# auduno/headtrackr

Hardware: AMD Instinct MI355X
Metric: frames/sec full-cascade detect at 320x240 (higher is better)
Workload: dtype u8; 1 GPU; C2: 256 x 320x240 RGBA frames per GPU, full BBF cascade detect (interval 5) incl. grouping + best face per frame on the host; frames_per_gpu=256, frames_total=256, width=320, height=240, batches_in_flight=3, parallelism=1 GPU

## Files before the change

headtrackr_amd/csrc/ht_context.hip:

```cpp
#include <sched.h>
#include <algorithm>
#include <cmath>
#include <cstddef>
#include <cstdlib>
#include <cstring>
#include <new>

#include "ht_internal.h"
#include "ht_hostpost.h"
#include "ht_geometry_plan.h"
#include "ht_cascade_plan.h"

static thread_local std::string g_create_err;

#include <dlfcn.h>
namespace {
struct Roctx {
    int (*push)(const char *) = nullptr;
    int (*pop)() = nullptr;
    Roctx() {
        void *h = dlopen("libroctx64.so", RTLD_NOW | RTLD_GLOBAL);
        if (!h) h = dlopen("libroctx64.so.4", RTLD_NOW | RTLD_GLOBAL);
        if (h) {
            push = reinterpret_cast<int (*)(const char *)>(dlsym(h, "roctxRangePushA"));
// ... 69 lines not shown
        int cpus = sched_getaffinity(0, sizeof(set), &set) == 0 ? CPU_COUNT(&set) : (int)std::thread::hardware_concurrency();
        int ngpu = 1;
        if (hipGetDeviceCount(&ngpu) != hipSuccess || ngpu < 1) ngpu = 1;
        return std::max(0, std::min(7, cpus / (2 * ngpu) - 1));
    }();
    return share;
}


ht_status ht_fail(ht_ctx *ctx, ht_status st, const std::string &msg) {
    if (ctx)
        ctx->err = msg;
    else
        g_create_err = msg;
    return st;
}

HtProfScope::HtProfScope(ht_ctx *c, const char *name, hipStream_t on) : ctx(c), stream(on ? on : c->stream) {
    if (!ctx->profiling) return;
    for (size_t i = 0; i < ctx->timers.size(); i++)
        if (ctx->timers[i].name == name) idx = (int)i;
    if (idx < 0) {
        ctx->timers.emplace_back();
        ctx->timers.back().name = name;
        idx = (int)ctx->timers.size() - 1;
    }
    if (hipEventCreate(&a) != hipSuccess || hipEventCreate(&b) != hipSuccess) {
        idx = -1;
        return;
    }
    (void)hipEventRecord(a, stream);
}
HtProfScope::~HtProfScope() {
    if (idx < 0) return;
    (void)hipEventRecord(b, stream);
    ctx->timers[idx].pending.emplace_back(a, b);
    ctx->timers[idx].launches++;
}

extern "C" int32_t ht_abi_version(void) { return HT_ABI_VERSION; }

extern "C" const char *ht_last_error(const ht_ctx *ctx) { return ctx ? ctx->err.c_str() : g_create_err.c_str(); }

static bool apply_options(ht_ctx *c, const std::string &opts, std::string &why) {
    size_t pos = 0;
    while (pos < opts.size()) {
        size_t end = opts.find(',', pos);
        if (end == std::string::npos) end = opts.size();
        std::string kv = opts.substr(pos, end - pos);
        pos = end + 1;
        while (!kv.empty() && (kv.front() == ' ')) kv.erase(kv.begin());
        while (!kv.empty() && (kv.back() == ' ')) kv.pop_back();
        if (kv.empty()) continue;
        const size_t eq = kv.find('=');
        const std::string key = kv.substr(0, eq), val = eq == std::string::npos ? "1" : kv.substr(eq + 1);
        char *endp = nullptr;
        const long long v = std::strtoll(val.c_str(), &endp, 10);
        if (val.empty() || (endp && *endp)) {
            why = "option '" + key + "': value is not an integer";
            return false;
        }
        const int iv = (int)std::max<long long>(std::min<long long>(v, 1ll << 30), -(1ll << 30));
        if (key == "rs_rpt") { if (iv >= 1 && iv <= HT_RS_MAX_PASSES) c->rs_rpt = iv; }
        else if (key == "rs_tailtable") c->tail_table = iv < 0 ? 0 : (iv > 2 ? 2 : (int)iv), c->tail_table_forced = true;
        else if (key == "rs_tailcap") c->rs_tailcap = (uint64_t)std::max<long long>(v, 0), c->rs_tailcap_forced = true;
        else if (key == "rs_notail") c->rs_notail = iv != 0;
        else if (key == "rs_nofast") c->rs_nofast = iv != 0;
        else if (key == "rs_nosort") c->rs_nosort = iv != 0;
        else if (key == "rs_bands") c->rs_bands = iv != 0;
        else if (key == "rs_gennames") c->rs_gennames = iv != 0;
        else if (key == "rs_minwg") c->rs_min_wgs = std::max(1, iv);
        else if (key == "rs_k") c->dbg_rs_k = iv;
        else if (key == "rs_group") { if (iv >= 1 && iv <= 64) c->rs_group = iv, c->rs_group_forced = true; }
        else if (key == "early_scan") c->early_scan = iv != 0;
        else if (key == "force_exact") c->dbg_force_exact = iv;
        else if (key == "deep_bias") c->deep_bias = (uint32_t)std::max(0, iv);
        else if (key == "deep_v") c->dbg_deep_v = iv;
        else if (key == "cs_flags") c->cs_flags = iv != 0;
        else if (key == "cs_sync_ring") c->cs_sync_ring = iv != 0;
        else if (key == "cs_pairs_force") c->cs_pairs_force = iv != 0;
        else if (key == "cs_pairs_cluster") c->cs_pairs_cluster = iv != 0;
        else if (key == "fp_sparse") c->fp_sparse = iv != 0;
        else if (key == "deep_grid") c->deep_grid = std::max(1, iv);
        else if (key == "split") c->opt_split = std::max(1, iv);
        else if (key == "cs_fused_min") c->cs_fused_min_streams = std::max(1, iv);
        else if (key == "cs_fused_nt") c->cs_fused_nt = iv;
        else if (key == "cs_keep_hist") c->cs_keep_hist = iv != 0;
        else if (key == "cs_seq_fused") c->cs_seq_fused = iv != 0;
        else if (key == "cs_cluster") c->cs_cluster = iv != 0;
        else if (key == "cs_cluster_min_px") c->cs_cluster_min_px = (uint32_t)std::max(0, iv);
        else if (key == "cs_region") c->cs_region_cap = std::min(40960, std::max(0, iv));
        else if (key == "cs_barrier_budget") c->cs_barrier_budget = std::max(1ll, v);
        else if (key == "graph_max_frames") c->graph_max_frames = std::max(0, iv);
        else if (key == "host_threads") c->host_threads = std::min(64, std::max(0, iv));
        else if (key == "force_rccl") c->force_rccl = iv != 0;
        else if (key == "group_cap") c->grp_cap_opt = std::max(1, iv);
#ifdef HT_DEBUG_KNOBS
        else if (key == "stop_stage") c->dbg_stop_stage = iv;
        else if (key == "cs_iters") c->dbg_cs_iters = std::min(10, std::max(0, iv));
        else if (key == "rs_maxgen") c->rs_maxgen = iv;
#endif
        else {
            why = "unknown option '" + key + "'";
            return false;
        }
    }
    return true;
}

template <typename T>
static ht_status upload_table(ht_ctx *c, T *&dst, const std::vector<T> &src) {
    if (src.empty()) return HT_OK;
    HT_HIP(c, hipMalloc(&dst, src.size() * sizeof(T)));
    HT_HIP(c, hipMemcpy(dst, src.data(), src.size() * sizeof(T), hipMemcpyHostToDevice));
    return HT_OK;
}

extern "C" ht_status ht_create(const ht_config *cfg, const void *cascade_blob, size_t cascade_len, ht_ctx **out) {
    if (!cfg || !out || (cfg->struct_size != sizeof(ht_config) && cfg->struct_size != offsetof(ht_config, options)))
        return ht_fail(nullptr, HT_ERR_INVALID, "ht_create: bad config");
    *out = nullptr;
    if (cfg->interval < 1 || cfg->interval > 12) return ht_fail(nullptr, HT_ERR_INVALID, "ht_create: interval must be 1..12");
    int ndev = 0;
    if (hipGetDeviceCount(&ndev) != hipSuccess || ndev <= 0)
        return ht_fail(nullptr, HT_ERR_NO_DEVICE, "ht_create: no HIP device visible (this library has no CPU fallback)");
    if (cfg->device < 0 || cfg->device >= ndev) return ht_fail(nullptr, HT_ERR_INVALID, "ht_create: device ordinal out of range");
    hipDeviceProp_t prop;
    if (hipGetDeviceProperties(&prop, cfg->device) != hipSuccess) return ht_fail(nullptr, HT_ERR_HIP, "hipGetDeviceProperties failed");
    if (std::strncmp(prop.gcnArchName, "gfx950", 6) != 0)
        return ht_fail(nullptr, HT_ERR_NO_DEVICE, std::string("ht_create: device is ") + prop.gcnArchName + ", this build is gfx950-only");
    ht_ctx *c = new (std::nothrow) ht_ctx();
    if (!c) return ht_fail(nullptr, HT_ERR_NOMEM, "ht_create: out of host memory");
    c->device = cfg->device;
    c->num_cus = prop.multiProcessorCount > 0 ? prop.multiProcessorCount : 256;
    c->interval = cfg->interval;
    c->next = cfg->interval + 1;
    if (cfg->hit_capacity) c->hit_capacity = cfg->hit_capacity;
    c->queue_capacity_cfg = cfg->queue_capacity;
    std::string why;
    if (!ht_plan_cascade((const uint8_t *)cascade_blob, cascade_len, &c->cascade, &why)) {
        delete c;
        return ht_fail(nullptr, HT_ERR_INVALID, "ht_create: " + why);
    }
    ht_status st = HT_OK;
    auto bail = [&](ht_status s) {
        g_create_err = c->err;
        ht_destroy(c);
        return s;
    };
    if (hipSetDevice(c->device) != hipSuccess) {
        c->err = "hipSetDevice failed";
        return bail(HT_ERR_HIP);
    }
    if (cfg->stream) {
        c->stream = (hipStream_t)cfg->stream;
    } else {
        if (hipStreamCreateWithFlags(&c->stream, hipStreamNonBlocking) != hipSuccess) {
            c->err = "hipStreamCreate failed";
            return bail(HT_ERR_HIP);
        }
        c->own_stream = true;
    }
    {
        std::string opts = (cfg->struct_size >= offsetof(ht_config, options) + sizeof(const char *) && cfg->options) ? cfg->options : "";
#ifdef HT_DEBUG_KNOBS
        if (const char *e = std::getenv("HT_OPTIONS")) opts += std::string(opts.empty() ? "" : ",") + e;
// ... 798 lines not shown
```

headtrackr_amd/csrc/ht_internal.h:

```cpp
#pragma once

#include <hip/hip_runtime.h>
#include <stdint.h>

#include <atomic>
#include <string>
#include <vector>

#include "headtrackr_hip.h"

#include "ht_cascade_types.h"

#include "ht_plan_types.h"

constexpr int HT_TAIL_LDS_TAPS = 4096;

struct HtBlockRef {
    uint16_t item;
    uint16_t bx, by;
    uint16_t pad;
};

struct alignas(16) HtQueueEntry {
    uint32_t frame;
    uint16_t x, y;
    uint8_t scale, q;
    uint16_t stage;
    uint32_t o0, o1, o2;
    uint16_t s0, s1, s2;
    uint16_t pad;
};
static_assert(sizeof(HtQueueEntry) == 32, "HtQueueEntry");

#define HT_DEEP_CTRS 16
#define HT_DEEP_CTR_BYTES (HT_DEEP_CTRS * 256)
#define HT_PINNED_HITS 8192
#define HT_STAT_SHARDS 256

struct HtCounters {
    uint32_t nhits;
    uint32_t nqueue;
    uint32_t queue_inline;
    uint32_t pad;
};

#include "ht_cs_schedule.h"

struct HtDetectGraph {
    const uint8_t *frames = nullptr;
    size_t frame_stride = 0;
    int nframes = 0;
    uint32_t flags = 0;
    int seen = 0;
    hipGraph_t graph = nullptr;
    hipGraphExec_t exec = nullptr;
};

struct HtKernelTimer {
    std::string name;
    double ms = 0;
    uint32_t launches = 0;
    std::vector<std::pair<hipEvent_t, hipEvent_t>> pending;
};

struct ht_ctx {
    int device = 0;
    hipStream_t stream = nullptr;
    bool own_stream = false;
    hipStream_t aux_stream = nullptr;
    hipEvent_t ev_early_ready = nullptr, ev_early_done = nullptr;
    bool early_scan = false;
    bool early_launched = false;
    std::string err;

    int interval = 5, next = 6;
    HtCascadePlan cascade;
    HtTileFeature *d_tile_feats = nullptr;
    HtDeepFeature *d_deep_feats = nullptr;
    HtPatchFeature *d_patch_feats = nullptr;
    HtPackedFeature *d_packed_feats = nullptr;
    HtPackedFeature *d_fp_feats = nullptr;
    bool fp_sparse = true;
    bool builtin_cascade = false;
    uint32_t deep_bias = 1;
    int dbg_stop_stage = -1, dbg_force_exact = 0, dbg_deep_v = 4, deep_grid = 192;
    HtDevStage *d_stages = nullptr;
    int opt_split = 0;

    int W = 0, H = 0, max_batch = 0, nlevels = 0, upto = 0;
    HtGeometryPlan plan;
    HtDevLevel *d_levels = nullptr;
    uint8_t *d_arena = nullptr;
    std::vector<HtResampleJob *> d_gen_blocks;
    HtTileRec *d_tile_recs = nullptr;
    HtScanScale *d_scales = nullptr;
    HtResampleJob *d_tail_jobs = nullptr;
    uint32_t *d_tail_prefix = nullptr;
    HtTap *d_tail_taps = nullptr;
    HtTapFast *d_tail_taps_fast = nullptr;
    HtTailTapRef *d_tail_tapref = nullptr;
    bool deep_attr_set = false;
    int tail_table = 1;
    bool tail_table_forced = false;
    bool rs_nofast = false, rs_nosort = false, rs_notail = false, rs_gennames = false;
    uint64_t rs_tailcap = 32768;
    bool rs_tailcap_forced = false;
    int rs_maxgen = 1 << 30;
    bool force_rccl = false;
    int host_threads = -1;
    int rs_min_wgs = 1536;
    int dbg_rs_k = 0;
    int rs_group = 8;
    bool rs_group_forced = false;
    int rs_rpt = 4;
    bool rs_bands = true;

    uint8_t *d_frames_own = nullptr;
    size_t d_frames_own_bytes = 0;
    uint8_t *d_frames_back = nullptr;
    size_t d_frames_back_bytes = 0;
    int back_n = 0;
    hipStream_t copy_stream = nullptr;
    hipEvent_t ev_copy_done = nullptr, ev_front_free = nullptr;
    const uint8_t *d_frames = nullptr;
    size_t frame_stride = 0;
    int nframes = 0;
    std::atomic<bool> capturing{false};
    int graph_max_frames = 256;
    std::vector<HtDetectGraph> graphs;
    uint64_t graph_launches = 0;
    int64_t requeue_flags = -1;
    int enq_nframes = 0;

    uint32_t hit_capacity = 1u << 20, queue_capacity_cfg = 0;
    ht_hit *d_hits = nullptr;
    HtQueueEntry *d_queue = nullptr;
    HtCounters *d_counters = nullptr;
    uint32_t spec_hint = 0;
    HtCounters h_counters;
    uint8_t *h_pinned = nullptr;
    unsigned long long *d_stats = nullptr;
    unsigned long long h_stage_in[64] = {0};
    std::vector<ht_hit> h_collect_hits;
    std::vector<uint32_t> h_collect_counts;
    std::vector<ht_hit> h_raw_hits;
    std::vector<ht_hit> h_ordered_hits;
    std::vector<uint32_t> h_frame_start;
    bool stats_enqueued = false;
    bool enqueued = false;
    bool collect_best_follows = false;
    bool h_sort_deferred = false;

    double *d_scratch = nullptr;
    size_t d_scratch_bytes = 0;
    bool wb_fused = false;
    bool wb_enqueued = false;
    unsigned long long *h_wb_pinned = nullptr;
    size_t h_wb_pinned_bytes = 0;
    std::vector<unsigned long long> h_wb_sums;
    int wb_collected_n = -1;

    int cs_streams = 0;
    HtCsState *d_cs = nullptr;
    uint32_t *d_cs_hist = nullptr;
    ht_cs_trackobj *d_cs_out = nullptr;
    double *d_cs_lut = nullptr, *d_cs_parts = nullptr;
    bool cs_cluster = true;
    uint32_t cs_cluster_min_px = 10000;
// ... 168 lines not shown
```

headtrackr_amd/csrc/ht_scan.hip:

```cpp
#include <algorithm>
#include <cmath>
#include <cstdlib>
#include <cstring>

#include "ht_internal.h"

namespace {

constexpr int TXH = HT_SCAN_TXH;
constexpr int TYH = HT_SCAN_TYH;
constexpr int NT = 256;
constexpr int TILE_WPS = 6;
constexpr int PITCH0 = HT_SCAN_PITCH0;
static_assert(PITCH0 >= 2 * TXH + 24 && PITCH0 % 8 == 0, "PITCH0");
constexpr int ROWS0 = HT_SCAN_ROWS0;
constexpr int P0_BYTES = PITCH0 * ROWS0;
constexpr int GH = HT_SCAN_GH;
constexpr int G_PITCH = HT_SCAN_G_PITCH;
constexpr int P12_BASE = HT_SCAN_P12_BASE;
constexpr int LDS_TILE_BYTES = HT_SCAN_LDS_TILE_BYTES;
constexpr int MAXWIN = TXH * TYH;
static_assert(P0_BYTES % 16 == 0 && P12_BASE == P0_BYTES, "alignment");

#include "ht_cascade_gen.inc"

__device__ __forceinline__ uint32_t lane_id() { return __builtin_amdgcn_mbcnt_hi(~0u, __builtin_amdgcn_mbcnt_lo(~0u, 0u)); }

#define HT_OFF(tab, j) (((j) & 1) ? ((tab)[(j) >> 1] >> 16) : ((tab)[(j) >> 1] & 0xffffu))
#define HT_RD(tab, j) ((uint32_t)lds[B + HT_OFF(tab, j)])

__device__ __forceinline__ double eval_stage_lds(const uint8_t *lds, uint32_t B, const HtTileFeature *__restrict__ F, uint32_t count) {
    double sum = 0.0;
    for (uint32_t k = 0; k < count; k++) {
        const uint4 P4 = *reinterpret_cast<const uint4 *>(F[k].po);
        const uint4 N4 = *reinterpret_cast<const uint4 *>(F[k].no);
        const uint4 A4 = *reinterpret_cast<const uint4 *>(F[k].a);
        const uint32_t np = F[k].np, nn = F[k].nn;
        const uint32_t po[4] = {P4.x, P4.y, P4.z, P4.w}, no[4] = {N4.x, N4.y, N4.z, N4.w};
        uint32_t pmin = HT_RD(po, 0), nmax = HT_RD(no, 0);
        if (np > 1) {
            pmin = min(pmin, HT_RD(po, 1));
            if (np > 2) {
                pmin = min(pmin, HT_RD(po, 2));
                if (np > 3) {
                    pmin = min(pmin, HT_RD(po, 3));
                    if (np > 4) {
                        pmin = min(pmin, HT_RD(po, 4));
                        if (np > 5) {
                            pmin = min(pmin, HT_RD(po, 5));
                            if (np > 6) {
                                pmin = min(pmin, HT_RD(po, 6));
                                if (np > 7) pmin = min(pmin, HT_RD(po, 7));
                            }
                        }
                    }
                }
            }
        }
        if (nn > 1) {
            nmax = max(nmax, HT_RD(no, 1));
            if (nn > 2) {
                nmax = max(nmax, HT_RD(no, 2));
                if (nn > 3) {
                    nmax = max(nmax, HT_RD(no, 3));
                    if (nn > 4) {
                        nmax = max(nmax, HT_RD(no, 4));
                        if (nn > 5) {
                            nmax = max(nmax, HT_RD(no, 5));
                            if (nn > 6) {
                                nmax = max(nmax, HT_RD(no, 6));
                                if (nn > 7) nmax = max(nmax, HT_RD(no, 7));
                            }
                        }
                    }
                }
            }
        }
        const bool fire = pmin > nmax;
        sum = __dadd_rn(sum, __hiloint2double((int)(fire ? A4.w : A4.y), (int)(fire ? A4.z : A4.x)));
    }
    return sum;
}

#ifdef HT_TILE_TIMELINE
#define TL_STAMP(p)                                                                              \
    do {                                                                                         \
        __builtin_amdgcn_sched_barrier(0);                                                       \
        if (my_stats && tid == 0) {                                                              \
// ... 520 lines not shown
            }
#pragma unroll
            for (int k = 0; k < 5; k++) {
                const uint32_t i = lane + 64u * k;
                if (i < 288u) *reinterpret_cast<uint16_t *>(&patch[2u * i]) = (uint16_t)pa[k];
            }
#pragma unroll
            for (int k = 0; k < 3; k++) {
                const uint32_t i = lane + 64u * k;
                if (i < 144u) patch[PATCH1 + i] = (uint8_t)pb[k];
            }
            if (lane < 36u) patch[PATCH2 + lane] = (uint8_t)pc;
        }
        __builtin_amdgcn_fence(__ATOMIC_RELEASE, "wavefront");
        __builtin_amdgcn_wave_barrier();
        bool alive = true;
        double conf = 0.0;
        uint32_t kb = 0;
        long long acc = 0;
        while (true) {
            const bool stage_ends = kb + 64u >= st.count;
            int jn = j;
            uint32_t kbn = kb + 64u;
            HtDevStage stn = st;
            if (stage_ends) {
                jn = j + 1;
                kbn = 0;
                if (jn < nstages) stn = stages[jn];
            }
            PatchFeatRegs nxt = cur;
            if (jn < nstages && kbn + lane < stn.count) nxt = load_feat(feats + stn.first + kbn + lane);
            if (kb == 0 && lane == 0 && my_stats) atomicAdd(&my_stats[j], 1ull);
            if (use_int) {
                if (kb + lane < st.count) acc += fire_regs(patch, cur, st.maxpts) ? cur.a1i : cur.a0i;
            }
            if (stage_ends) {
                bool need_exact = true;
                if (use_int) {
                    const long long Ssum = wave_sum_i64(acc);
                    acc = 0;
                    if (Ssum < st.thri) {
                        alive = false;
                        break;
                    }
                    need_exact = (Ssum == st.thri) || (j == nstages - 1) || use_int == 2;
                }
                if (need_exact) {
                    const double sum = patch_stage_sum_exact(patch, feats + st.first, st.count, st.maxpts, lane);
                    if (sum < st.threshold) {
                        alive = false;
                        break;
                    }
                    conf = sum;
                }
                if (jn >= nstages) break;
            }
            j = jn;
            kb = kbn;
            st = stn;
            cur = nxt;
        }
        if (alive && lane == 0) {
            if (my_stats) atomicAdd(&my_stats[nstages], 1ull);
            const uint32_t pos = atomicAdd(&ctr->nhits, 1u);
            if (pos < hit_cap) {
                ht_hit h;
                h.frame = ent.frame;
                h.x = ent.x;
                h.y = ent.y;
                h.scale = ent.scale;
                h.q = ent.q;
                h.reserved0 = 0;
                h.reserved1 = 0;
                h.sum = conf;
                hits[pos] = h;
            }
        }
        __builtin_amdgcn_wave_barrier();
    }
}

constexpr uint32_t DEEP_LDS_TABLE_BYTES = HT_DEEP_LDS_TABLE_BYTES;
constexpr int DEEPL_WAVES = 12;
static_assert(DEEP_LDS_TABLE_BYTES + 64 * sizeof(HtDevStage) + DEEPL_WAVES * (PATCH_BYTES + 512) <= 96 * 1024, "the largest packed tail the planner builds fits the dynamic LDS ht_launch_scan asks for");

__device__ __forceinline__ bool packed_fire(const uint8_t *patch, const uint4 A, const uint32_t B0) {
    const uint32_t p0 = A.x & 0xffffu, p1 = A.x >> 16, p2 = A.y & 0xffffu, p3 = A.y >> 16, p4 = A.z & 0xffffu;
    const uint32_t n0 = A.z >> 16, n1 = A.w & 0xffffu, n2 = A.w >> 16, n3 = B0 & 0xffffu, n4 = B0 >> 16;
    const uint32_t pmin = min(min(min((uint32_t)patch[p0], (uint32_t)patch[p1]), min((uint32_t)patch[p2], (uint32_t)patch[p3])), (uint32_t)patch[p4]);
    const uint32_t nmax = max(max(max((uint32_t)patch[n0], (uint32_t)patch[n1]), max((uint32_t)patch[n2], (uint32_t)patch[n3])), (uint32_t)patch[n4]);
    return pmin > nmax;
}

__device__ __forceinline__ int wave_sum_i32_dpp(int v) {
    int s = v + __builtin_amdgcn_update_dpp(0, v, 0x111, 0xf, 0xf, true);
    s += __builtin_amdgcn_update_dpp(0, v, 0x112, 0xf, 0xf, true);
    s += __builtin_amdgcn_update_dpp(0, v, 0x113, 0xf, 0xf, true);
    s += __builtin_amdgcn_update_dpp(0, s, 0x114, 0xf, 0xe, true);
    s += __builtin_amdgcn_update_dpp(0, s, 0x118, 0xf, 0xc, true);
    s += __builtin_amdgcn_update_dpp(0, s, 0x142, 0xa, 0xf, true);
    s += __builtin_amdgcn_update_dpp(0, s, 0x143, 0xc, 0xf, true);
    return __builtin_amdgcn_readlane(s, 63);
}
__device__ __forceinline__ long long wave_sum_i64_dpp(long long v) {
    const unsigned long long u = (unsigned long long)(v + (1ll << 40));
    const long long l0 = wave_sum_i32_dpp((int)(u & 0x1fffffu));
    const long long l1 = wave_sum_i32_dpp((int)((u >> 21) & 0x1fffffu));
    const long long l2 = wave_sum_i32_dpp((int)(u >> 42));
    return l0 + (l1 << 21) + (l2 << 42) - (64ll << 40);
}

struct DeepEntry {
    uint32_t frame, x, y, scale, q, stage, o0, o1, o2, s0, s1, s2;
};
__device__ __forceinline__ DeepEntry deep_entry(const HtQueueEntry *__restrict__ queue, uint32_t e) {
    typedef unsigned int u32x4 __attribute__((ext_vector_type(4)));
    typedef const __attribute__((address_space(4))) u32x4 *cptr4;
    cptr4 p = (cptr4)(reinterpret_cast<uintptr_t>(queue) + (uintptr_t)e * sizeof(HtQueueEntry));
    const u32x4 w0 = p[0], w1 = p[1];
    DeepEntry d;
    d.frame = w0.x, d.x = w0.y & 0xffffu, d.y = w0.y >> 16;
    d.scale = w0.z & 0xffu, d.q = (w0.z >> 8) & 0xffu, d.stage = w0.z >> 16;
    d.o0 = w0.w, d.o1 = w1.x, d.o2 = w1.y;
    d.s0 = w1.z & 0xffffu, d.s1 = w1.z >> 16, d.s2 = w1.w & 0xffffu;
    return d;
}

#ifdef HT_DEEP_TIMELINE
__device__ unsigned long long g_deep_tl[8192][8];
#define DL_STAMP(i)                                                                                                  \
    do {                                                                                                             \
        __builtin_amdgcn_sched_barrier(0);                                                                           \
        if ((threadIdx.x & 63u) == 0 && dl_first) g_deep_tl[(blockIdx.x * DEEPL_WAVES + (threadIdx.x >> 6)) & 8191u][i] = __builtin_readcyclecounter(); \
        __builtin_amdgcn_sched_barrier(0);                                                                           \
    } while (0)
#else
#define DL_STAMP(i)
#endif
__global__ __launch_bounds__(64 * DEEPL_WAVES, (2 * DEEPL_WAVES + 3) / 4) void k_scan_deep_lds(const uint8_t *__restrict__ arena, uint64_t arena_stride,
                                                                   const HtDevLevel *__restrict__ levels, int next,
                                                                   const HtPackedFeature *__restrict__ packed, uint32_t packed_count,
                                                                   uint32_t packed_first, const HtDevStage *__restrict__ stages, int nstages,
                                                                   int force_exact, const HtQueueEntry *__restrict__ queue, uint32_t queue_cap,
                                                                   ht_hit *__restrict__ hits, uint32_t hit_cap, HtCounters *__restrict__ ctr,
                                                                   unsigned long long *__restrict__ stats) {
    extern __shared__ __attribute__((aligned(16))) uint8_t dyn_lds[];
    uint4 *tab = reinterpret_cast<uint4 *>(dyn_lds);
    HtDevStage *s_stages = reinterpret_cast<HtDevStage *>(dyn_lds + (size_t)packed_count * sizeof(HtPackedFeature));
    uint8_t *per_wave = reinterpret_cast<uint8_t *>(s_stages + 64);
    const uint32_t n = min(ctr->nqueue, queue_cap);
    if (blockIdx.x * DEEPL_WAVES >= n) return;
#ifdef HT_DEEP_TIMELINE
    bool dl_first = true;
#endif
    DL_STAMP(0);
    const uint32_t lane = threadIdx.x & 63u, wv = (uint32_t)__builtin_amdgcn_readfirstlane((int)(threadIdx.x >> 6));
    const uint32_t wave = blockIdx.x * DEEPL_WAVES + wv, nwaves = (uint32_t)__builtin_amdgcn_readfirstlane((int)(gridDim.x * DEEPL_WAVES));
    DeepEntry ent = deep_entry(queue, min(wave, n - 1u));
    {
        typedef __attribute__((address_space(3))) void lds_void;
        typedef const __attribute__((address_space(1))) void glb_void;
        const uint32_t tab_bytes = packed_count * (uint32_t)sizeof(HtPackedFeature);
        for (uint32_t c0 = wv * 1024u; c0 < tab_bytes; c0 += DEEPL_WAVES * 1024u) {
            const uint32_t off = c0 + lane * 16u;
            if (off < tab_bytes)
                __builtin_amdgcn_global_load_lds((glb_void *)(reinterpret_cast<const uint8_t *>(packed) + off), (lds_void *)(dyn_lds + c0), 16, 0, 0);
        }
    }
    for (uint32_t i = threadIdx.x; i < (uint32_t)nstages * (sizeof(HtDevStage) / 16); i += blockDim.x)
        reinterpret_cast<uint4 *>(s_stages)[i] = reinterpret_cast<const uint4 *>(stages)[i];
    bool table_published = false;
    uint8_t *patch = per_wave + wv * (PATCH_BYTES + 512);
    double *sel_buf = reinterpret_cast<double *>(patch + PATCH_BYTES);
    unsigned long long *my_stats = stats ? stats + (size_t)(wave & (HT_STAT_SHARDS - 1)) * 64 : nullptr;
    const uint32_t *my_ctr = reinterpret_cast<const uint32_t *>(queue + queue_cap) + (wave & (HT_DEEP_CTRS - 1u)) * 64u;
    for (uint32_t e = wave; e < n;) {
        e = (uint32_t)__builtin_amdgcn_readfirstlane((int)e);
        uint32_t nxt = 0;
        if (lane == 0) {
            const uint32_t zero = 0u, one = 1u;
            asm volatile("global_atomic_add %0, %1, %2, %3 sc0" : "=v"(nxt) : "v"(zero), "v"(one), "s"(my_ctr) : "memory");
        }
        uint32_t ln = lane;
        asm volatile("" : "+v"(ln));
        const uint8_t *fb = arena + (uint64_t)ent.frame * arena_stride;
        const uint32_t o0 = ent.o0, o1 = ent.o1, o2 = ent.o2;
        const int s0 = (int)ent.s0, s1 = (int)ent.s1, s2 = (int)ent.s2;
        const DeepEntry cur = ent;
        uint32_t e_next;
        {
            uint32_t pa[5], pb[3], pc = 0;
#pragma unroll
            for (int k = 0; k < 5; k++) {
                const uint32_t i = ln + 64u * k, r = i / 12u, c2 = (i - r * 12u) * 2u;
                pa[k] = 0;
                if (i < 288u) pa[k] = *reinterpret_cast<const uint16_t *>(fb + o0 + r * (uint32_t)s0 + c2);
            }
#pragma unroll
            for (int k = 0; k < 3; k++) {
                const uint32_t i = ln + 64u * k, r = i / 12u, c = i - r * 12u;
                pb[k] = 0;
                if (i < 144u) pb[k] = fb[o1 + r * (uint32_t)s1 + c];
            }
            if (ln < 36u) {
                const uint32_t r = ln / 6u, c = ln - r * 6u;
                pc = fb[o2 + r * (uint32_t)s2 + c];
            }
#pragma unroll
            for (int k = 0; k < 5; k++) {
                const uint32_t i = ln + 64u * k;
                if (i < 288u) *reinterpret_cast<uint16_t *>(&patch[2u * i]) = (uint16_t)pa[k];
            }
#pragma unroll
            for (int k = 0; k < 3; k++) {
                const uint32_t i = ln + 64u * k;
                if (i < 144u) patch[PATCH1 + i] = (uint8_t)pb[k];
            }
            if (ln < 36u) patch[PATCH2 + ln] = (uint8_t)pc;
            static_assert(PATCH2 + 36 <= 760 && PATCH_BYTES >= 764, "spare bytes of the patch");
            if (lane == 0) asm volatile("s_waitcnt vmcnt(0)" : "+v"(nxt) : : "memory");
            e_next = nwaves + HT_DEEP_CTRS * (uint32_t)__builtin_amdgcn_readlane((int)nxt, 0) + (wave & (HT_DEEP_CTRS - 1u));
            if (e_next < n) ent = deep_entry(queue, e_next);
        }
        __builtin_amdgcn_fence(__ATOMIC_RELEASE, "wavefront");
        __builtin_amdgcn_wave_barrier();
        if (!table_published) {
            __builtin_amdgcn_s_waitcnt(0x0f70);
            __syncthreads();
            table_published = true;
            DL_STAMP(1);
        }
        DL_STAMP(2);
        bool alive = true;
        double conf = 0.0;
        for (int j = (int)cur.stage; j < nstages; j++) {
            const HtDevStage st = s_stages[j];
            const uint32_t base = st.first - packed_first;
            if (lane == 0 && my_stats) atomicAdd(&my_stats[j], 1ull);
            long long acc = 0;
            constexpr int KEEP = 10;
            int32_t kept[KEEP];
            const bool keep = (j == nstages - 1) && st.count <= 64u * KEEP;
            if (keep) {
#pragma unroll
                for (int cki = 0; cki < KEEP; cki++) {
                    const uint32_t k = 64u * cki + lane;
                    kept[cki] = 0;
                    if (64u * cki < st.count && k < st.count) {
                        const uint4 A = tab[(base + k) * 2u], Bq = tab[(base + k) * 2u + 1u];
                        kept[cki] = packed_fire(patch, A, Bq.x) ? (int32_t)Bq.z : (int32_t)Bq.y;
                        acc += (long long)kept[cki];
                    }
                    __builtin_amdgcn_sched_barrier(0);
                }
            } else {
                for (uint32_t k = lane; k < st.count; k += 64) {
                    const uint4 A = tab[(base + k) * 2u], Bq = tab[(base + k) * 2u + 1u];
                    acc += packed_fire(patch, A, Bq.x) ? (long long)(int32_t)Bq.z : (long long)(int32_t)Bq.y;
                }
            }
            const long long Ssum = wave_sum_i64_dpp(acc);
            if (Ssum < st.thri) {
                alive = false;
                break;
            }
#ifdef HT_DEEP_TIMELINE
            if (lane == 0 && dl_first) g_deep_tl[(blockIdx.x * DEEPL_WAVES + wv) & 8191u][4] = (unsigned long long)j;
#endif
            if (Ssum == st.thri || j == nstages - 1 || force_exact) {
                DL_STAMP(5);
                double sum = 0.0;
                auto sel_of = [&](uint32_t k) -> double {
                    double sel = 0.0;
                    if (k < st.count) {
                        const uint4 A = tab[(base + k) * 2u], Bq = tab[(base + k) * 2u + 1u];
                        const int32_t ai = packed_fire(patch, A, Bq.x) ? (int32_t)Bq.z : (int32_t)Bq.y;
                        sel = (double)ai / 1e8;
                    }
                    return sel;
                };
                auto add64 = [&](double sel) {
                    sel_buf[lane] = sel;
                    __builtin_amdgcn_fence(__ATOMIC_RELEASE, "wavefront");
                    __builtin_amdgcn_wave_barrier();
                    double g[8], h[8];
#pragma unroll
                    for (int u = 0; u < 8; u++) g[u] = sel_buf[u];
#pragma unroll
                    for (int grp = 0; grp < 8; grp++) {
                        if (grp < 7) {
#pragma unroll
                            for (int u = 0; u < 8; u++) h[u] = sel_buf[8 * (grp + 1) + u];
                        }
                        __builtin_amdgcn_sched_barrier(0);
#pragma unroll
                        for (int u = 0; u < 8; u++) sum = __dadd_rn(sum, g[u]);
#pragma unroll
                        for (int u = 0; u < 8; u++) g[u] = h[u];
                    }
                    __builtin_amdgcn_wave_barrier();
                };
                if (keep) {
#pragma unroll
                    for (int cki = 0; cki < KEEP; cki++)
                        if (64u * cki < st.count) add64((double)kept[cki] / 1e8);
                } else {
                    for (uint32_t kb = 0; kb < st.count; kb += 64) add64(sel_of(kb + lane));
                }
                if (sum < st.threshold) {
                    alive = false;
                    break;
                }
                conf = sum;
            }
        }
        if (alive && lane == 0) {
            if (my_stats) atomicAdd(&my_stats[nstages], 1ull);
            const uint32_t pos = atomicAdd(&ctr->nhits, 1u);
            if (pos < hit_cap) {
                ht_hit h;
                h.frame = cur.frame;
                h.x = (uint16_t)cur.x;
                h.y = (uint16_t)cur.y;
                h.scale = (uint8_t)cur.scale;
                h.q = (uint8_t)cur.q;
                h.reserved0 = 0;
                h.reserved1 = 0;
                h.sum = conf;
                hits[pos] = h;
            }
        }
        DL_STAMP(3);
#ifdef HT_DEEP_TIMELINE
        dl_first = false;
#endif
        __builtin_amdgcn_wave_barrier();
        e = e_next;
    }
    if (!table_published) {
        __builtin_amdgcn_s_waitcnt(0x0f70);
        __syncthreads();
    }
}


__global__ __launch_bounds__(256) void k_scan_simple(const uint8_t *__restrict__ arena, uint64_t arena_stride,
                                                     const HtDevLevel *__restrict__ levels, int next,
                                                     const HtScanScale *__restrict__ scales, int nscales, uint32_t windows_per_frame,
                                                     const HtDeepFeature *__restrict__ feats, const HtDevStage *__restrict__ stages,
                                                     int nstages, ht_hit *__restrict__ hits, uint32_t hit_cap,
                                                     HtCounters *__restrict__ ctr, unsigned long long *__restrict__ stats) {
    unsigned long long *my_stats = stats ? stats + (size_t)(blockIdx.x & (HT_STAT_SHARDS - 1)) * 64 : nullptr;
    const uint32_t wi = blockIdx.x * blockDim.x + threadIdx.x;
    const uint32_t frame = blockIdx.y;
    const uint32_t lane = threadIdx.x & 63u;
    bool alive = wi < windows_per_frame;
    int si = 0;
    for (int k = 1; k < nscales; k++)
        if (wi >= scales[k].win_begin) si = k;
    const HtScanScale S = scales[si];
    const uint32_t li = alive ? wi - S.win_begin : 0u;
    const uint32_t per = (uint32_t)(S.qw * S.qh);
    const uint32_t q = li / per, r = li - q * per, y = r / (uint32_t)S.qw, x = r - y * (uint32_t)S.qw;
    HT_WIN_SETUP(arena + (uint64_t)frame * arena_stride, levels, next, (uint32_t)S.l0, q, x, y)
    double sum = 0.0;
    for (int j = 0; j < nstages; j++) {
        const unsigned long long m = __ballot(alive);
        if (!m) break;
        if (lane == 0 && my_stats) atomicAdd(&my_stats[j], (unsigned long long)__popcll(m));
        const HtDevStage st = stages[j];
        const HtDeepFeature *F = feats + st.first;
        sum = 0.0;
        if (alive) {
            for (uint32_t k = 0; k < st.count; k++) {
                const HtDeepFeature &f = F[k];
                sum = __dadd_rn(sum, deep_fire(&f, HT_WIN_PASS, st.maxpts) ? f.a1 : f.a0);
            }
            if (sum < st.threshold) alive = false;
        }
    }
    if (alive) {
        if (my_stats) atomicAdd(&my_stats[nstages], 1ull);
        const uint32_t pos = atomicAdd(&ctr->nhits, 1u);
        if (pos < hit_cap) {
            ht_hit h;
            h.frame = frame;
            h.x = (uint16_t)x;
            h.y = (uint16_t)y;
            h.scale = (uint8_t)S.l0;
            h.q = (uint8_t)q;
            h.reserved0 = 0;
            h.reserved1 = 0;
            h.sum = sum;
            hits[pos] = h;
        }
    }
}

}


bool ht_scan_is_builtin_cascade(const uint8_t *blob, size_t len) {
    if (len != HT_GEN_CASCADE_LEN) return false;
    unsigned long long h = 0xcbf29ce484222325ull;
    for (size_t i = 0; i < len; i++) h = (h ^ blob[i]) * 0x100000001b3ull;
    return h == HT_GEN_CASCADE_FNV;
}

static ht_status launch_tiles(ht_ctx *c, uint32_t flags, hipStream_t stream, uint32_t first, uint32_t count) {
    unsigned long long *stats = (flags & HT_SCAN_STATS) ? c->d_stats : nullptr;
    const int split = (flags & HT_SCAN_NO_SPLIT) ? (int)c->cascade.nstages : (int)std::min<uint32_t>(c->cascade.split_stage, c->cascade.nstages);
    const uint64_t total64 = (uint64_t)count * (uint64_t)c->nframes;
    if (total64 > 0x7fffff00ull) return ht_fail(c, HT_ERR_INVALID, "ht_detect: batch too large for one launch");
    const uint32_t total = (uint32_t)total64;
    const bool gen = c->builtin_cascade && !(flags & HT_SCAN_GENERIC);
    const int stop_stage = c->dbg_stop_stage, force_exact = c->dbg_force_exact;
    HtProfScope ps(c, "scan_tiles", stream);
    if (gen)
        hipLaunchKernelGGL(k_scan_tiles<true>, dim3((total + 7u) & ~7u), dim3(NT), 0, stream, c->d_arena, c->plan.arena_stride,
                           c->d_tile_recs + first, c->d_tile_feats, c->fp_sparse ? c->d_fp_feats : nullptr, c->d_stages, (int)c->cascade.nstages, split, c->deep_bias, stop_stage, force_exact, count, total,
                           c->d_queue, c->plan.queue_capacity, c->d_hits, c->hit_capacity, c->d_counters, stats);
    else
        hipLaunchKernelGGL(k_scan_tiles<false>, dim3((total + 7u) & ~7u), dim3(NT), 0, stream, c->d_arena, c->plan.arena_stride,
                           c->d_tile_recs + first, c->d_tile_feats, c->fp_sparse ? c->d_fp_feats : nullptr, c->d_stages, (int)c->cascade.nstages, split, c->deep_bias, stop_stage, force_exact, count, total,
                           c->d_queue, c->plan.queue_capacity, c->d_hits, c->hit_capacity, c->d_counters, stats);
    HT_HIP(c, hipGetLastError());
    return HT_OK;
}

ht_status ht_launch_scan_early(ht_ctx *c, uint32_t flags) {
    if (c->plan.early_tiles == 0 || !c->aux_stream || (flags & HT_SCAN_SIMPLE) || c->cascade.cw != 24 || c->cascade.ch != 24) return HT_OK;
    HT_HIP(c, hipEventRecord(c->ev_early_ready, c->stream));
    HT_HIP(c, hipStreamWaitEvent(c->aux_stream, c->ev_early_ready, 0));
    ht_status st = launch_tiles(c, flags, c->aux_stream, 0, c->plan.early_tiles);
    if (st != HT_OK) return st;
    HT_HIP(c, hipEventRecord(c->ev_early_done, c->aux_stream));
    c->early_launched = true;
    return HT_OK;
}

ht_status ht_launch_scan(ht_ctx *c, uint32_t flags) {
    if (c->plan.scales.empty() || c->plan.tiles_per_frame == 0) return HT_OK;
    const int nscales = (int)c->plan.scales.size();
    unsigned long long *stats = (flags & HT_SCAN_STATS) ? c->d_stats : nullptr;
    const bool tile_ok = (c->cascade.cw == 24 && c->cascade.ch == 24);
    if ((flags & HT_SCAN_SIMPLE) || !tile_ok) {
        HtProfScope ps(c, "scan_simple");
        dim3 grid((uint32_t)((c->plan.windows_per_frame + 255) / 256), c->nframes);
        hipLaunchKernelGGL(k_scan_simple, grid, dim3(256), 0, c->stream, c->d_arena, c->plan.arena_stride, c->d_levels, c->next, c->d_scales,
                           nscales, (uint32_t)c->plan.windows_per_frame, c->d_deep_feats, c->d_stages, (int)c->cascade.nstages, c->d_hits,
                           c->hit_capacity, c->d_counters, stats);
        HT_HIP(c, hipGetLastError());
        return HT_OK;
    }
    const int split = (flags & HT_SCAN_NO_SPLIT) ? (int)c->cascade.nstages : (int)std::min<uint32_t>(c->cascade.split_stage, c->cascade.nstages);
    const int force_exact = c->dbg_force_exact;
    {
        const uint32_t first = c->early_launched ? c->plan.early_tiles : 0u;
        ht_status st = launch_tiles(c, flags, c->stream, first, c->plan.tiles_per_frame - first);
        if (st != HT_OK) return st;
        if (c->early_launched) HT_HIP(c, hipStreamWaitEvent(c->stream, c->ev_early_done, 0));
    }
    if (split < (int)c->cascade.nstages) {
        HtProfScope ps(c, "scan_deep");
        const int deep_v = c->dbg_deep_v;
        if (deep_v == 4 && !c->cascade.packed.empty() && c->cascade.stages[split].first >= c->cascade.packed_first) {
            const size_t lds = c->cascade.packed.size() * sizeof(HtPackedFeature) + 64 * sizeof(HtDevStage) + (size_t)DEEPL_WAVES * (PATCH_BYTES + 512);
            if (!c->deep_attr_set) {
                HT_HIP(c, hipFuncSetAttribute(reinterpret_cast<const void *>(k_scan_deep_lds), hipFuncAttributeMaxDynamicSharedMemorySize, 96 * 1024));
                c->deep_attr_set = true;
            }
            const uint32_t deep_grid = std::max<uint32_t>((uint32_t)c->deep_grid, (HT_DEEP_CTRS + DEEPL_WAVES - 1) / DEEPL_WAVES);
            hipLaunchKernelGGL(k_scan_deep_lds, dim3(deep_grid), dim3(64 * DEEPL_WAVES), lds, c->stream, c->d_arena, c->plan.arena_stride, c->d_levels, c->next,
                               c->d_packed_feats, (uint32_t)c->cascade.packed.size(), c->cascade.packed_first, c->d_stages, (int)c->cascade.nstages, force_exact, c->d_queue, c->plan.queue_capacity,
                               c->d_hits, c->hit_capacity, c->d_counters, stats);
        } else
        hipLaunchKernelGGL(k_scan_deep, dim3(2048), dim3(64 * DEEP_WAVES), 0, c->stream, c->d_arena, c->plan.arena_stride, c->d_levels, c->next,
                           c->d_patch_feats, c->d_stages, (int)c->cascade.nstages, c->cascade.decimal_alphas ? (force_exact ? 2 : 1) : 0, c->d_queue, c->plan.queue_capacity, c->d_hits,
                           c->hit_capacity, c->d_counters, stats);
        HT_HIP(c, hipGetLastError());
    }
    return HT_OK;
}

#ifdef HT_DEEP_TIMELINE
extern "C" int ht_debug_deep_timeline(unsigned long long *out, int nmax) {
    static unsigned long long h[8192][8];
    if (hipMemcpyFromSymbol(h, HIP_SYMBOL(g_deep_tl), sizeof(h)) != hipSuccess) return -1;
    const int n = std::min(nmax, 8192);
    std::memcpy(out, h, (size_t)n * 8 * sizeof(unsigned long long));
    std::memset(h, 0, sizeof(h));
    if (hipMemcpyToSymbol(HIP_SYMBOL(g_deep_tl), h, sizeof(h)) != hipSuccess) return -1;
    return n;
}
#endif
```

Measured before the change: 1.126 million frames/s.

## Defer last-stage exact double sums to a block-wide pending pass

```diff
diff --git a/headtrackr_amd/csrc/ht_context.hip b/headtrackr_amd/csrc/ht_context.hip
--- a/headtrackr_amd/csrc/ht_context.hip
+++ b/headtrackr_amd/csrc/ht_context.hip
@@ -175,6 +175,7 @@
         else if (key == "cs_pairs_cluster") c->cs_pairs_cluster = iv != 0;
         else if (key == "fp_sparse") c->fp_sparse = iv != 0;
         else if (key == "deep_grid") c->deep_grid = std::max(1, iv);
+        else if (key == "deep_pend") c->deep_pend = std::min(HT_DEEP_PEND_MAX, std::max(0, iv));
         else if (key == "split") c->opt_split = std::max(1, iv);
         else if (key == "cs_fused_min") c->cs_fused_min_streams = std::max(1, iv);
         else if (key == "cs_fused_nt") c->cs_fused_nt = iv;
diff --git a/headtrackr_amd/csrc/ht_deep_sum.h b/headtrackr_amd/csrc/ht_deep_sum.h
--- /dev/null
+++ b/headtrackr_amd/csrc/ht_deep_sum.h
@@ -0,0 +1,56 @@
+#pragma once
+
+#include <stdint.h>
+
+#ifndef HT_DSUM_FN
+#define HT_DSUM_FN inline
+#endif
+#ifndef HT_DSUM_ADD
+#define HT_DSUM_ADD(a, b) ((a) + (b))
+#endif
+#ifndef HT_DSUM_SCHED
+#define HT_DSUM_SCHED()
+#endif
+
+constexpr uint32_t HT_DSUM_MAX_CHUNKS = 10;
+
+struct alignas(16) HtAlphaPair {
+    double a0, a1;
+};
+
+HT_DSUM_FN double ht_dsum_select(uint64_t mask_word, uint32_t bit, const HtAlphaPair &pair) { return ((mask_word >> bit) & 1u) ? pair.a1 : pair.a0; }
+
+HT_DSUM_FN uint32_t ht_dsum_row(uint32_t count) { return count | 1u; }
+
+HT_DSUM_FN double ht_dsum_seq(const double *t, uint32_t count) {
+    const uint32_t nsteps = count / 8u;
+    double sum = 0.0;
+    if (nsteps) {
+        double ta[8], tb[8];
+#define HT_DSUM_READ(r, sn)                                                                      \
+    do {                                                                                         \
+        _Pragma("GCC unroll 8") for (uint32_t u = 0; u < 8u; u++) r[u] = t[8u * (sn) + u];       \
+        HT_DSUM_SCHED();                                                                         \
+    } while (0)
+#define HT_DSUM_ADD8(r) _Pragma("GCC unroll 8") for (uint32_t u = 0; u < 8u; u++) sum = HT_DSUM_ADD(sum, r[u])
+        HT_DSUM_READ(ta, 0u);
+        uint32_t sn = 1;
+        for (; sn + 1u < nsteps; sn += 2u) {
+            HT_DSUM_READ(tb, sn);
+            HT_DSUM_ADD8(ta);
+            HT_DSUM_READ(ta, sn + 1u);
+            HT_DSUM_ADD8(tb);
+        }
+        if (sn < nsteps) {
+            HT_DSUM_READ(tb, sn);
+            HT_DSUM_ADD8(ta);
+            HT_DSUM_ADD8(tb);
+        } else {
+            HT_DSUM_ADD8(ta);
+        }
+#undef HT_DSUM_READ
+#undef HT_DSUM_ADD8
+    }
+    for (uint32_t k = 8u * nsteps; k < count; k++) sum = HT_DSUM_ADD(sum, t[k]);
+    return sum;
+}
diff --git a/headtrackr_amd/csrc/ht_internal.h b/headtrackr_amd/csrc/ht_internal.h
--- a/headtrackr_amd/csrc/ht_internal.h
+++ b/headtrackr_amd/csrc/ht_internal.h
@@ -34,6 +34,7 @@
 
 #define HT_DEEP_CTRS 16
 #define HT_DEEP_CTR_BYTES (HT_DEEP_CTRS * 256)
+#define HT_DEEP_PEND_MAX 32
 #define HT_PINNED_HITS 8192
 #define HT_STAT_SHARDS 256
 
@@ -83,7 +84,8 @@
     bool fp_sparse = true;
     bool builtin_cascade = false;
     uint32_t deep_bias = 1;
-    int dbg_stop_stage = -1, dbg_force_exact = 0, dbg_deep_v = 4, deep_grid = 192;
+    int dbg_stop_stage = -1, dbg_force_exact = 0, dbg_deep_v = 4, deep_grid = 160;
+    int deep_pend = HT_DEEP_PEND_MAX;
     HtDevStage *d_stages = nullptr;
     int opt_split = 0;
 
diff --git a/headtrackr_amd/csrc/ht_scan.hip b/headtrackr_amd/csrc/ht_scan.hip
--- a/headtrackr_amd/csrc/ht_scan.hip
+++ b/headtrackr_amd/csrc/ht_scan.hip
@@ -4,6 +4,11 @@
 #include <cstring>
 
 #include "ht_internal.h"
+
+#define HT_DSUM_FN __device__ __forceinline__
+#define HT_DSUM_ADD(a, b) __dadd_rn((a), (b))
+#define HT_DSUM_SCHED() __builtin_amdgcn_sched_barrier(0)
+#include "ht_deep_sum.h"
 
 namespace {
 
@@ -690,7 +695,19 @@
 
 constexpr uint32_t DEEP_LDS_TABLE_BYTES = HT_DEEP_LDS_TABLE_BYTES;
 constexpr int DEEPL_WAVES = 12;
-static_assert(DEEP_LDS_TABLE_BYTES + 64 * sizeof(HtDevStage) + DEEPL_WAVES * (PATCH_BYTES + 512) <= 96 * 1024, "the largest packed tail the planner builds fits the dynamic LDS ht_launch_scan asks for");
+struct alignas(16) DeepPending {
+    unsigned long long mask[HT_DSUM_MAX_CHUNKS];
+    uint32_t frame, xy, scale_q, pad;
+};
+constexpr uint32_t DEEP_PEND_MAX = HT_DEEP_PEND_MAX, DEEP_PEND_HEAD = 16;
+static_assert(sizeof(DeepPending) == 96 && DEEP_PEND_MAX <= 64, "one pending window per lane of the tail's wavefront");
+constexpr size_t DEEPL_BASE_LDS = 64 * sizeof(HtDevStage) + DEEPL_WAVES * (PATCH_BYTES + 512);
+static_assert(DEEP_LDS_TABLE_BYTES + DEEPL_BASE_LDS + DEEP_PEND_HEAD + DEEP_PEND_MAX * sizeof(DeepPending) <= 96 * 1024, "the largest packed tail the planner builds fits the dynamic LDS ht_launch_scan asks for");
+static size_t deepl_pend_cap(size_t packed_bytes, uint32_t wanted) {
+    const size_t base = packed_bytes + DEEPL_BASE_LDS, budget = base <= 80 * 1024 ? 80 * 1024 : 96 * 1024;
+    const size_t fit = base + DEEP_PEND_HEAD >= budget ? 0 : (budget - base - DEEP_PEND_HEAD) / sizeof(DeepPending);
+    return std::min<size_t>(std::min<size_t>(wanted, DEEP_PEND_MAX), fit);
+}
 
 __device__ __forceinline__ bool packed_fire(const uint8_t *patch, const uint4 A, const uint32_t B0) {
     const uint32_t p0 = A.x & 0xffffu, p1 = A.x >> 16, p2 = A.y & 0xffffu, p3 = A.y >> 16, p4 = A.z & 0xffffu;
@@ -742,22 +759,33 @@
         if ((threadIdx.x & 63u) == 0 && dl_first) g_deep_tl[(blockIdx.x * DEEPL_WAVES + (threadIdx.x >> 6)) & 8191u][i] = __builtin_readcyclecounter(); \
         __builtin_amdgcn_sched_barrier(0);                                                                           \
     } while (0)
+__device__ unsigned long long g_deep_tail[1024][4];
+#define DL_TAIL(i, v)                                                                  \
+    do {                                                                               \
+        __builtin_amdgcn_sched_barrier(0);                                             \
+        if (threadIdx.x == 0) g_deep_tail[blockIdx.x & 1023u][i] = (v);                \
+        __builtin_amdgcn_sched_barrier(0);                                             \
+    } while (0)
 #else
 #define DL_STAMP(i)
+#define DL_TAIL(i, v)
 #endif
 __global__ __launch_bounds__(64 * DEEPL_WAVES, (2 * DEEPL_WAVES + 3) / 4) void k_scan_deep_lds(const uint8_t *__restrict__ arena, uint64_t arena_stride,
                                                                    const HtDevLevel *__restrict__ levels, int next,
                                                                    const HtPackedFeature *__restrict__ packed, uint32_t packed_count,
                                                                    uint32_t packed_first, const HtDevStage *__restrict__ stages, int nstages,
-                                                                   int force_exact, const HtQueueEntry *__restrict__ queue, uint32_t queue_cap,
+                                                                   int force_exact, uint32_t pend_cap, const HtQueueEntry *__restrict__ queue, uint32_t queue_cap,
                                                                    ht_hit *__restrict__ hits, uint32_t hit_cap, HtCounters *__restrict__ ctr,
                                                                    unsigned long long *__restrict__ stats) {
     extern __shared__ __attribute__((aligned(16))) uint8_t dyn_lds[];
     uint4 *tab = reinterpret_cast<uint4 *>(dyn_lds);
     HtDevStage *s_stages = reinterpret_cast<HtDevStage *>(dyn_lds + (size_t)packed_count * sizeof(HtPackedFeature));
     uint8_t *per_wave = reinterpret_cast<uint8_t *>(s_stages + 64);
+    uint32_t *pend_n = reinterpret_cast<uint32_t *>(per_wave + DEEPL_WAVES * (PATCH_BYTES + 512));
+    DeepPending *pend = reinterpret_cast<DeepPending *>(reinterpret_cast<uint8_t *>(pend_n) + DEEP_PEND_HEAD);
     const uint32_t n = min(ctr->nqueue, queue_cap);
     if (blockIdx.x * DEEPL_WAVES >= n) return;
+    if (pend_cap && threadIdx.x == 0) *pend_n = 0u;
 #ifdef HT_DEEP_TIMELINE
     bool dl_first = true;
 #endif
@@ -846,19 +874,20 @@
             const uint32_t base = st.first - packed_first;
             if (lane == 0 && my_stats) atomicAdd(&my_stats[j], 1ull);
             long long acc = 0;
-            constexpr int KEEP = 10;
-            int32_t kept[KEEP];
+            constexpr int KEEP = (int)HT_DSUM_MAX_CHUNKS;
+            uint32_t fired = 0u;
             const bool keep = (j == nstages - 1) && st.count <= 64u * KEEP;
             if (keep) {
 #pragma unroll
                 for (int cki = 0; cki < KEEP; cki++) {
                     const uint32_t k = 64u * cki + lane;
-                    kept[cki] = 0;
+                    bool fire = false;
                     if (64u * cki < st.count && k < st.count) {
                         const uint4 A = tab[(base + k) * 2u], Bq = tab[(base + k) * 2u + 1u];
-                        kept[cki] = packed_fire(patch, A, Bq.x) ? (int32_t)Bq.z : (int32_t)Bq.y;
-                        acc += (long long)kept[cki];
+                        fire = packed_fire(patch, A, Bq.x);
+                        acc += fire ? (long long)(int32_t)Bq.z : (long long)(int32_t)Bq.y;
                     }
+                    fired |= (uint32_t)fire << cki;
                     __builtin_amdgcn_sched_barrier(0);
                 }
             } else {
@@ -875,6 +904,24 @@
 #ifdef HT_DEEP_TIMELINE
             if (lane == 0 && dl_first) g_deep_tl[(blockIdx.x * DEEPL_WAVES + wv) & 8191u][4] = (unsigned long long)j;
 #endif
+            if (keep && !force_exact) {
+                uint32_t slot = pend_cap;
+                if (pend_cap) {
+                    if (lane == 0) slot = atomicAdd(pend_n, 1u);
+                    slot = (uint32_t)__builtin_amdgcn_readfirstlane((int)slot);
+                }
+                if (slot < pend_cap) {
+                    DeepPending *pe = pend + slot;
+#pragma unroll
+                    for (int cki = 0; cki < KEEP; cki++) {
+                        const unsigned long long fm = __ballot((fired >> cki) & 1u);
+                        if (lane == 0) pe->mask[cki] = fm;
+                    }
+                    if (lane == 0) pe->frame = cur.frame, pe->xy = cur.x | (cur.y << 16), pe->scale_q = cur.scale | (cur.q << 8), pe->pad = 0u;
+                    alive = false;
+                    break;
+                }
+            }
             if (Ssum == st.thri || j == nstages - 1 || force_exact) {
                 DL_STAMP(5);
                 double sum = 0.0;
@@ -911,7 +958,15 @@
                 if (keep) {
 #pragma unroll
                     for (int cki = 0; cki < KEEP; cki++)
-                        if (64u * cki < st.count) add64((double)kept[cki] / 1e8);
+                        if (64u * cki < st.count) {
+                            const uint32_t k = 64u * cki + lane;
+                            double sel = 0.0;
+                            if (k < st.count) {
+                                const uint4 Bq = tab[(base + k) * 2u + 1u];
+                                sel = (double)(((fired >> cki) & 1u) ? (int32_t)Bq.z : (int32_t)Bq.y) / 1e8;
+                            }
+                            add64(sel);
+                        }
                 } else {
                     for (uint32_t kb = 0; kb < st.count; kb += 64) add64(sel_of(kb + lane));
                 }
@@ -949,6 +1004,55 @@
         __builtin_amdgcn_s_waitcnt(0x0f70);
         __syncthreads();
     }
+    if (pend_cap == 0u) return;
+    __syncthreads();
+    const uint32_t asked = *pend_n, m = min(asked, pend_cap);
+    DL_TAIL(0, __builtin_readcyclecounter());
+    DL_TAIL(2, (unsigned long long)asked);
+    DL_TAIL(3, (unsigned long long)pend_cap);
+    if (m == 0u) {
+        DL_TAIL(1, __builtin_readcyclecounter());
+        return;
+    }
+    static_assert(64 * HT_DSUM_MAX_CHUNKS <= 64 * DEEPL_WAVES, "a thread per feature of the last stage");
+    const HtDevStage stl = s_stages[nstages - 1];
+    HtAlphaPair mine = {0.0, 0.0};
+    if (threadIdx.x < stl.count) {
+        const uint4 Bq = tab[(stl.first - packed_first + threadIdx.x) * 2u + 1u];
+        mine.a0 = (double)(int32_t)Bq.y / 1e8, mine.a1 = (double)(int32_t)Bq.z / 1e8;
+    }
+    double *rows = reinterpret_cast<double *>(dyn_lds);
+    const uint32_t row = ht_dsum_row(stl.count);
+    const uint32_t per_round = min(packed_count * (uint32_t)sizeof(HtPackedFeature) / (row * (uint32_t)sizeof(double)), 64u);
+    for (uint32_t w0 = 0; w0 < m; w0 += per_round) {
+        const uint32_t nw = min(m - w0, per_round);
+        __syncthreads();
+        if (threadIdx.x < stl.count)
+            for (uint32_t w = 0; w < nw; w++)
+                rows[w * row + threadIdx.x] = ht_dsum_select(pend[w0 + w].mask[wv], lane, mine);
+        __syncthreads();
+        if (threadIdx.x < nw) {
+            const DeepPending *pe = pend + w0 + threadIdx.x;
+            const double sum = ht_dsum_seq(rows + threadIdx.x * row, stl.count);
+            if (!(sum < stl.threshold)) {
+                if (my_stats) atomicAdd(&my_stats[nstages], 1ull);
+                const uint32_t pos = atomicAdd(&ctr->nhits, 1u);
+                if (pos < hit_cap) {
+                    ht_hit h;
+                    h.frame = pe->frame;
+                    h.x = (uint16_t)(pe->xy & 0xffffu);
+                    h.y = (uint16_t)(pe->xy >> 16);
+                    h.scale = (uint8_t)(pe->scale_q & 0xffu);
+                    h.q = (uint8_t)(pe->scale_q >> 8);
+                    h.reserved0 = 0;
+                    h.reserved1 = 0;
+                    h.sum = sum;
+                    hits[pos] = h;
+                }
+            }
+        }
+    }
+    DL_TAIL(1, __builtin_readcyclecounter());
 }
 
 
@@ -1073,14 +1177,16 @@
         HtProfScope ps(c, "scan_deep");
         const int deep_v = c->dbg_deep_v;
         if (deep_v == 4 && !c->cascade.packed.empty() && c->cascade.stages[split].first >= c->cascade.packed_first) {
-            const size_t lds = c->cascade.packed.size() * sizeof(HtPackedFeature) + 64 * sizeof(HtDevStage) + (size_t)DEEPL_WAVES * (PATCH_BYTES + 512);
+            const size_t packed_bytes = c->cascade.packed.size() * sizeof(HtPackedFeature);
+            const uint32_t pend_cap = (uint32_t)deepl_pend_cap(packed_bytes, (uint32_t)c->deep_pend);
+            const size_t lds = packed_bytes + DEEPL_BASE_LDS + (pend_cap ? DEEP_PEND_HEAD + pend_cap * sizeof(DeepPending) : 0);
             if (!c->deep_attr_set) {
                 HT_HIP(c, hipFuncSetAttribute(reinterpret_cast<const void *>(k_scan_deep_lds), hipFuncAttributeMaxDynamicSharedMemorySize, 96 * 1024));
                 c->deep_attr_set = true;
             }
             const uint32_t deep_grid = std::max<uint32_t>((uint32_t)c->deep_grid, (HT_DEEP_CTRS + DEEPL_WAVES - 1) / DEEPL_WAVES);
             hipLaunchKernelGGL(k_scan_deep_lds, dim3(deep_grid), dim3(64 * DEEPL_WAVES), lds, c->stream, c->d_arena, c->plan.arena_stride, c->d_levels, c->next,
-                               c->d_packed_feats, (uint32_t)c->cascade.packed.size(), c->cascade.packed_first, c->d_stages, (int)c->cascade.nstages, force_exact, c->d_queue, c->plan.queue_capacity,
+                               c->d_packed_feats, (uint32_t)c->cascade.packed.size(), c->cascade.packed_first, c->d_stages, (int)c->cascade.nstages, force_exact, pend_cap, c->d_queue, c->plan.queue_capacity,
                                c->d_hits, c->hit_capacity, c->d_counters, stats);
         } else
         hipLaunchKernelGGL(k_scan_deep, dim3(2048), dim3(64 * DEEP_WAVES), 0, c->stream, c->d_arena, c->plan.arena_stride, c->d_levels, c->next,
@@ -1101,4 +1207,13 @@
     if (hipMemcpyToSymbol(HIP_SYMBOL(g_deep_tl), h, sizeof(h)) != hipSuccess) return -1;
     return n;
 }
+extern "C" int ht_debug_deep_tail(unsigned long long *out, int nmax) {
+    static unsigned long long h[1024][4];
+    if (hipMemcpyFromSymbol(h, HIP_SYMBOL(g_deep_tail), sizeof(h)) != hipSuccess) return -1;
+    const int n = std::min(nmax, 1024);
+    std::memcpy(out, h, (size_t)n * 4 * sizeof(unsigned long long));
+    std::memset(h, 0, sizeof(h));
+    if (hipMemcpyToSymbol(HIP_SYMBOL(g_deep_tail), h, sizeof(h)) != hipSuccess) return -1;
+    return n;
+}
 #endif
```

After: 1.137 million frames/s, median of 6. Within noise of the previous version (+1.0%).
